# renaudbedard/raytracing-in-one-weekend

Measured on AMD Instinct MI355X. Metric: Msamples/s, 486-sphere cover scene 1920x1080 8-bounce, higher is better.
Workload: dtype f32

## Files before the change

__graft_entry__.py:

```python
import importlib
import os
import subprocess
import sys

ROOT = os.path.dirname(os.path.abspath(__file__))
if ROOT not in sys.path:
    sys.path.insert(0, ROOT)


def build():
    csrc = os.path.join(ROOT, "raytracing-in-one-weekend_amd", "csrc")
    subprocess.run(["make", "-C", csrc], check=True)
    subprocess.run(["make", "-C", os.path.join(ROOT, "oracle")], check=True)
    out_dir = os.path.join(ROOT, "tests", "build")
    os.makedirs(out_dir, exist_ok=True)
    flags = ["-std=c++17", "-O3", "--offload-arch=gfx950", "-ffp-contract=off", "-fno-fast-math", "-Wno-unused-value", "-x", "hip"]
    for name in ("detmath_parity", "exactmath_parity", "exactdiv_parity", "finalize_parity"):
        src, exe = os.path.join(ROOT, "tests", "native", name + ".hip"), os.path.join(out_dir, name)
        deps = [src] + [os.path.join(csrc, h) for h in ("rtow_finalize.hip.h", "rtow_detmath.hip.h", "rtow_exactmath.hip.h")]
        if not os.path.exists(exe) or os.path.getmtime(exe) < max(os.path.getmtime(d) for d in deps):
            subprocess.run(["/opt/rocm/bin/hipcc"] + (flags if name != "detmath_parity" else ["-std=c++17", "-O2", "--offload-arch=gfx950", "-ffp-contract=off", "-fno-fast-math", "-x", "hip"]) + [src, "-o", exe], check=True)
    src, so = os.path.join(ROOT, "tests", "native", "hitsort_parity.hip"), os.path.join(out_dir, "libhitsort_parity.so")
    hdr = os.path.join(ROOT, "raytracing-in-one-weekend_amd", "csrc", "rtow_sample_kernel.hip.h")
    if not os.path.exists(so) or os.path.getmtime(so) < max(os.path.getmtime(src), os.path.getmtime(hdr)):
        subprocess.run(["/opt/rocm/bin/hipcc"] + flags[:-2] + ["-Wno-unused-function", "-fPIC", "-shared", "-x", "hip", src, "-o", so], check=True)
    src, so = os.path.join(ROOT, "tests", "native", "fake_rccl.cpp"), os.path.join(out_dir, "libfake_rccl.so")
    if not os.path.exists(so) or os.path.getmtime(so) < os.path.getmtime(src):
        subprocess.run(["/opt/rocm/bin/hipcc", "-std=c++17", "-O2", "-fPIC", "-shared", "-x", "c++", "-D__HIP_PLATFORM_AMD__", "-I/opt/rocm/include", src, "-o", so,
                        "-L/opt/rocm/lib", "-lamdhip64", "-pthread"], check=True)
    for name in ("valu_calib", "coherence_probe", "sqrt_variants", "xcd_affinity_probe"):
        src, exe = os.path.join(ROOT, "profiles", "calib", name + ".hip"), os.path.join(ROOT, "profiles", "calib", name)
        if not os.path.exists(exe) or os.path.getmtime(exe) < os.path.getmtime(src):
            subprocess.run(["/opt/rocm/bin/hipcc", "-O2"] + flags[2:] + [src, "-o", exe], check=True)
    rt = importlib.import_module("raytracing-in-one-weekend_amd")
    lib = rt.lib.load()
    assert lib.rtowGetApiVersion() == rt.abi.RTOW_API_VERSION
    for name in rt.abi.EXPORTED_SYMBOLS:
        getattr(lib, name)


def smoke():
    import numpy as np

    rt = importlib.import_module("raytracing-in-one-weekend_amd")
    from oracle import binding as ob

    scene = rt.scenes.cover_scene()
    desc = scene.desc()
    params = rt.scenes.make_params(scene, 96, 54, spp=4, trace_depth=8)
    with rt.Context(0) as ctx:
        ctx.upload_scene(desc)
        gpu = rt.sample_batch_host(ctx, params)
        ms = ctx.last_sample_kernel_ms()
    osc = ob.OracleScene(desc)
    ref = osc.sample_batch(params)
    osc.close()
    for k in ("color", "normal", "albedo", "scw"):
        assert np.array_equal(gpu[k].view(np.uint32), ref[k].view(np.uint32)), "smoke: %s differs from the oracle" % k
    assert np.array_equal(gpu["diag"][:, 0], ref["diag"][:, 0]), "smoke: RayCount differs"
    mean = gpu["color"][:, :3] / np.maximum(gpu["color"][:, 3:4], 1)
    mref = ref["color"][:, :3] / np.maximum(ref["color"][:, 3:4], 1)
    assert np.abs(mean - mref).max() <= 1e-4
    plist = [rt.scenes.make_params(scene, 96, 54, spp=4, trace_depth=8, seed=s) for s in (1, 2)]
    n = 96 * 54
    with rt.Context(0) as ctx:
        ctx.upload_scene(desc)
        bufs = [rt.DeviceBuffer(ctx, n * c * 4).zero() for c in (4, 3, 3, 1)]
        rt.lib.check(rt.sample_batch_chain_device(ctx, plist, bufs, bufs), "rtowSampleBatchChainDevice")
        ctx.synchronize()
        chained = {k: b.download(np.float32, (n, c)) for k, b, c in zip(("color", "normal", "albedo", "scw"), bufs, (4, 3, 3, 1))}
    osc = ob.OracleScene(desc)
    ref2 = osc.sample_batch(plist[1], {k: ref[k] for k in ("color", "normal", "albedo", "scw")})
    osc.close()
    for k in ("color", "normal", "albedo", "scw"):
        assert np.array_equal(chained[k].reshape(-1).view(np.uint32), ref2[k].reshape(-1).view(np.uint32)), "smoke: chained %s differs from the oracle" % k
    print("smoke ok: 96x54x4spp cover scene bit-exact vs oracle (single batch and a chain of two), kernel %.3f ms" % ms)


if __name__ == "__main__":
    build()
    if len(sys.argv) > 1 and sys.argv[1] == "smoke":
        smoke()
```

raytracing-in-one-weekend_amd/csrc/rtow_exactmath.hip.h:

```cpp
#pragma once
#include <hip/hip_runtime.h>

namespace rtow {

__device__ __forceinline__ float exact_rcp(float x)
{
    if (__builtin_expect(((__float_as_uint(x) & 0x7f800000u) - 0x01000000u) <= 0x7d000000u, 1)) {
        const float y = __builtin_amdgcn_rcpf(x);
        const float e = __builtin_fmaf(-x, y, 1.0f);
        return __builtin_fmaf(e, y, y);
    }
    return 1.0f / x;
}

__device__ __forceinline__ float exact_rcp_nan_to_inf(float x)
{
    if (__builtin_expect(((__float_as_uint(x) & 0x7f800000u) - 0x01000000u) <= 0x7d000000u, 1)) {
        const float y = __builtin_amdgcn_rcpf(x);
        const float e = __builtin_fmaf(-x, y, 1.0f);
        return __builtin_fmaf(e, y, y);
    }
    const float r = 1.0f / x;
    return r != r ? __builtin_inff() : r;
}

__device__ __forceinline__ float exact_sqrt(float x)
{
    if (__builtin_expect((__float_as_uint(x) - 0x10000000u) < 0x6f000000u, 1)) {
        const float y = __builtin_amdgcn_rsqf(x);
        const float s = x * y;
        const float h = 0.5f * y;
        const float r = __builtin_fmaf(-s, s, x);
        return __builtin_fmaf(r, h, s);
    }
    return __builtin_sqrtf(x);
}

__device__ __forceinline__ float exact_div_step(float a, float b, float y)
{
    const float q = a * y;
    const float r = __builtin_fmaf(-b, q, a);
    return __builtin_fmaf(r, y, q);
}

__device__ __forceinline__ void exact_div3(float ax, float ay, float az, float b, float& qx, float& qy, float& qz)
{
    const unsigned g = ((__float_as_uint(ax) << 1) + 0x40000000u) & ((__float_as_uint(ay) << 1) + 0x40000000u) & ((__float_as_uint(az) << 1) + 0x40000000u);
    const bool bOk = ((__float_as_uint(b) & 0x7f800000u) - 0x30000000u) < 0x20000000u;
    if (__builtin_expect((int)g < 0 && bOk, 1)) {
        const float y0 = __builtin_amdgcn_rcpf(b);
        const float e = __builtin_fmaf(-b, y0, 1.0f);
        const float y = __builtin_fmaf(e, y0, y0);
        qx = exact_div_step(ax, b, y);
        qy = exact_div_step(ay, b, y);
        qz = exact_div_step(az, b, y);
    } else {
        qx = ax / b; qy = ay / b; qz = az / b;
    }
}

__host__ inline float exact_rcp(float x) { return 1.0f / x; }
__host__ inline float exact_rcp_nan_to_inf(float x) { const float r = 1.0f / x; return r != r ? __builtin_inff() : r; }
__host__ inline float exact_sqrt(float x) { return __builtin_sqrtf(x); }
__host__ inline void exact_div3(float ax, float ay, float az, float b, float& qx, float& qy, float& qz) { qx = ax / b; qy = ay / b; qz = az / b; }

}
```

raytracing-in-one-weekend_amd/csrc/rtow_sample_kernel.hip.h:

```cpp
#pragma once
#include "rtow_kernels.h"

#include <type_traits>

#include "rtow_detmath.hip.h"
#include "rtow_hit_tests.hip.h"
#include "rtow_surface.hip.h"
#include "rtow_vecmath.hip.h"

#ifndef RTOW_WHOLE_MATERIAL
#define RTOW_WHOLE_MATERIAL 1
#endif
#ifndef RTOW_LDS_VIEW
#define RTOW_LDS_VIEW 2
#endif
#ifndef RTOW_COLD_VIEW
#define RTOW_COLD_VIEW 1
#endif
#ifndef RTOW_TRI_HOT
#define RTOW_TRI_HOT 1
#endif
#ifndef RTOW_PREFETCH
#define RTOW_PREFETCH 0
#endif
#ifndef RTOW_PINHOLE
#define RTOW_PINHOLE 1
#endif
#ifndef RTOW_TIE_WATCH
#define RTOW_TIE_WATCH 1
#endif

namespace rtow {

namespace {

__device__ __forceinline__ float inv_pow2(int depth)
{
    if (depth <= 126) return __uint_as_float((unsigned)(127 - depth) << 23);
    if (depth == 127) return __uint_as_float(0x00400000u);
    return 0.0f;
}

__device__ __forceinline__ float rng_next(unsigned& state)
{
    const unsigned t = state;
    unsigned s = t;
    s ^= s << 13;
    s ^= s >> 17;
    s ^= s << 5;
    state = s;
    return __uint_as_float(0x3f800000u | (t >> 9)) - 1.0f;
}

__device__ __forceinline__ V3 tangent_to_world(float tx, float ty, float tz, V3 n)
{
    const float s = n.z >= 0 ? 1.0f : -1.0f;
    const float a = -RTOW_RCP(s + n.z);
    const float b = n.x * n.y * a;
    const V3 tangent = v3(1 + s * n.x * n.x * a, s * b, -s * n.x);
    const V3 bitangent = v3(b, s + n.y * n.y * a, -n.y);
    const V3 r = v3(tangent.x * tx + n.x * ty + bitangent.x * tz,
                    tangent.y * tx + n.y * ty + bitangent.y * tz,
                    tangent.z * tx + n.z * ty + bitangent.z * tz);
    return normalize(r);
}
__device__ __forceinline__ V3 cosine_hemisphere_uv(float u, float v, V3 n)
{
    const float radius = RTOW_SQRT(u);
    const float theta = v * 2 * kPi;
    float sinT, cosT;
    det_sincos(theta, sinT, cosT);
    const float tx = radius * cosT, tz = radius * sinT;
    const float ty = RTOW_SQRT(1 - u);
    return tangent_to_world(tx, ty, tz, n);
}
__device__ __forceinline__ V3 direction_uv(float r0, float r1)
{
    const float z = r0 * 2.0f - 1.0f;
    const float rr = RTOW_SQRT(um_max(1.0f - z * z, 0.0f));
    const float angle = r1 * kPi * 2.0f;
    float sn, cs;
    det_sincos(angle, sn, cs);
    return v3(cs * rr, sn * rr, z);
}

struct NoiseSite { const SampleKernelArgs* A; unsigned cx, cy; };

__device__ __forceinline__ unsigned noise_texel(unsigned n, unsigned rowStride, unsigned cx, unsigned cy)
{
    constexpr float g = 1.32471795724474602596f;
    constexpr float a1 = 1.0f / g;
    constexpr float a2 = 1.0f / (g * g);
    const float fn = (float)(n - 1u);
    const float x = 0.5f + a1 * fn, y = 0.5f + a2 * fn;
    const float rx = x - __builtin_floorf(x), ry = y - __builtin_floorf(y);
    const unsigned ox = (unsigned)__builtin_floorf(rx * (float)rowStride), oy = (unsigned)__builtin_floorf(ry * (float)rowStride);
    return ((cy + oy) % rowStride) * rowStride + ((cx + ox) % rowStride);
}

template <int NOISE>
struct Rng;

template <>
struct Rng<RTOW_NOISE_WHITE> {
    unsigned s;
    __device__ __forceinline__ void begin_pixel(const NoiseSite&, unsigned pix, unsigned seed)
    {
        s = (seed * 0x8C4CA03Fu) ^ (pix * 0x7383ED49u);
        (void)rng_next(s);
    }
    __device__ __forceinline__ void begin_sample(const NoiseSite& at, unsigned pix, unsigned smp)
    {
        s = ((at.A->seed * 0x8C4CA03Fu) ^ (pix * 0x7383ED49u)) ^ ((smp + 1u) * 0x9E3779B9u);
        if (s == 0u) s = 0x9E3779B9u;
        (void)rng_next(s);
    }
    __device__ __forceinline__ float next(const NoiseSite&) { return rng_next(s); }
    __device__ __forceinline__ void next2(const NoiseSite&, float& a, float& b) { a = rng_next(s); b = rng_next(s); }
    __device__ __forceinline__ void in_unit_disk(const NoiseSite&, float& x, float& y)
    {
        const float theta = rng_next(s) * (2.0f * kPi - 0.0f) + 0.0f;
        const float radius = RTOW_SQRT(rng_next(s));
        float sinT, cosT;
        det_sincos(theta, sinT, cosT);
        x = radius * cosT; y = radius * sinT;
    }
    __device__ __forceinline__ V3 cosine_hemisphere(const NoiseSite&, V3 n) { const float u = rng_next(s), v = rng_next(s); return cosine_hemisphere_uv(u, v, n); }
    __device__ __forceinline__ void skip_cosine_hemisphere(const NoiseSite&) { (void)rng_next(s); (void)rng_next(s); }
    __device__ __forceinline__ V3 direction(const NoiseSite&) { const float r0 = rng_next(s), r1 = rng_next(s); return direction_uv(r0, r1); }
    __device__ __forceinline__ unsigned trace_value() const { return s; }
};

struct RngPerSample {
    unsigned s, s1;
    __device__ __forceinline__ static unsigned rotl(unsigned x, unsigned k) { return __builtin_amdgcn_alignbit(x, x, 32u - k); }
    __device__ __forceinline__ float draw(const NoiseSite& at)
    {
        if (at.A->xoroshiro) {
            const unsigned s0 = s;
            unsigned t1 = s1;
            const unsigned result = rotl(s0 * 0x9E3779BBu, 5u) * 5u;
            t1 ^= s0;
            s = rotl(s0, 26u) ^ t1 ^ (t1 << 9);
            s1 = rotl(t1, 13u);
            return __uint_as_float(0x3f800000u | (result >> 9)) - 1.0f;
        }
        return rng_next(s);
    }
    __device__ __forceinline__ void begin_pixel(const NoiseSite&, unsigned, unsigned) { s = 1u; s1 = 0u; }
    __device__ __forceinline__ void begin_sample(const NoiseSite& at, unsigned pix, unsigned smp)
    {
        s = ((at.A->seed * 0x8C4CA03Fu) ^ (pix * 0x7383ED49u)) ^ ((smp + 1u) * 0x9E3779B9u);
        if (at.A->xoroshiro) {
            s1 = (s * 0x85EBCA6Bu) ^ 0xC2B2AE35u;
            if ((s | s1) == 0u) s1 = 0x9E3779B9u;
        } else if (s == 0u) {
// ... 540 lines not shown
    int st = ST_REGEN;
    int pix = -1;
    unsigned tick = 0;
    typename std::conditional<PER_SAMPLE && NOISE == RTOW_NOISE_WHITE, RngPerSample, Rng<NOISE>>::type rng{};
    V3 fbNormal = v3(0, 0, 0), fbAlbedo = v3(0, 0, 0);
    unsigned unitGroup = 0;
    unsigned smp = 0, nsamp = 0;
    int cx = 0, cy = 0;
    V3 colorAcc = v3(0, 0, 0), normalAcc = v3(0, 0, 0), albedoAcc = v3(0, 0, 0);
    float scwAcc = 0, scw0 = 0;
    int sampleCount = 0;
    float rayCount = 0, boundsHits = 0, candidates = 0;

    V3 ro = v3(0, 0, 0), rd = v3(0, 0, 1);
    float rtime = 0;
    int depth = 0;
    Hist<HW> hist;
    hist.clear();
    V3 sampleNormal = v3(0, 0, 0);
    int firstNs = -1;
    float randomEventsLocal = 0;

    float texHist[TEXTURED ? HW * 2 * 6 : 1];
    constexpr int kMaxHits = VOLUMES ? kLocalHits : 1;
    float hitT[kMaxHits], hitTmin0[kMaxHits];
    unsigned hitCode[kMaxHits];
    bool tieAtBest = false;
    bool hitOverflow = false;
    int nHits = 0;
    int curVol = -1;
    float pendRE = 0;
    bool insideHit = false;
    float hitTmin = 0;
    constexpr bool TRIANGLES_ONLY = BASE == SCENE_KIND_TRIANGLES || BASE == SCENE_KIND_TRIANGLES_TEXTURED;
    constexpr bool TRI_HOT = TRIANGLES_ONLY && RTOW_TRI_HOT;
    constexpr bool PREFETCH_FAR = WIDE && !ALL_LDS && (RTOW_PREFETCH & 1) != 0;
    constexpr bool PREFETCH_TRI = WIDE && !ALL_LDS && TRI_HOT && (RTOW_PREFETCH & 2) != 0;
    const uint32_t ldsDump __attribute__((unused)) = (uint32_t)(uintptr_t)(__attribute__((address_space(3))) uint8_t*)(smem + ((uint32_t)kCandCapacity + A.ldsStackRows) * (uint32_t)BT * 4u);
    constexpr bool KEEP_NORMAL = BASE == SCENE_KIND_GENERAL || BASE == SCENE_KIND_TRIANGLES;
    V3 keptNormal = v3(0, 0, 0);

    V3 inv = v3(0, 0, 0);
    int cur = 0, sp = 0, nc = 0, prim = -1;
    float best = 0;

    auto endSample = [&](bool ok, V3 sampleColor, V3 skyColor) {
        V3 sampleAlbedo = ok ? skyColor : v3(0, 0, 0);
        if (firstNs >= 0) {
            const unsigned code = hist.get(firstNs, histRows);
            const bool white = (code & 0x8000u) != 0;
            if (TEXTURED) {
                const V3 refl = white ? v3(1, 1, 1) : v3(texHist[firstNs * 6 + 0], texHist[firstNs * 6 + 1], texHist[firstNs * 6 + 2]);
                sampleAlbedo = add(v3(texHist[firstNs * 6 + 3], texHist[firstNs * 6 + 4], texHist[firstNs * 6 + 5]), refl);
            } else {
                const uint8_t* mp = section<ALL_LDS>(sc, L.materialOffset) + (code & 0x7fffu) * 64u;
                const float4 m0 = *reinterpret_cast<const float4*>(mp);
                const float2 m1 = *reinterpret_cast<const float2*>(mp + 16);
                const V3 refl = white ? v3(1, 1, 1) : v3(m0.x, m0.y, m0.z);
                sampleAlbedo = add(v3(m0.w, m1.x, m1.y), refl);
            }
        }
        if (ok) {
            scwAcc += randomEventsLocal;
            colorAcc = add(colorAcc, sampleColor);
            normalAcc = add(normalAcc, sampleNormal);
            albedoAcc = add(albedoAcc, sampleAlbedo);
            sampleCount++;
        } else if (PER_SAMPLE) {
            if (smp == 0) { fbNormal = sampleNormal; fbAlbedo = sampleAlbedo; }
        } else if (smp == 0 && sampleCount == 0 && !A.probeOnly) {
            const SampleKernelArgs& R = A;
            float* fbN = R.outNormal;
            float* fbA = R.outAlbedo;
            if (chained && R.chainIndependent) { fbN = R.chainBatches[tick >> kChainShift].outNormal; fbA = R.chainBatches[tick >> kChainShift].outAlbedo; }
            fbN += 3 * (size_t)pix;
            fbA += 3 * (size_t)pix;
            fbN[0] = sampleNormal.x; fbN[1] = sampleNormal.y; fbN[2] = sampleNormal.z;
            fbA[0] = sampleAlbedo.x; fbA[1] = sampleAlbedo.y; fbA[2] = sampleAlbedo.z;
        }
        smp++;
        st = ST_REGEN;
    };
    auto startRay = [&]() {
        inv = v3(RTOW_RCP_NAN_TO_INF(rd.x), RTOW_RCP_NAN_TO_INF(rd.y), RTOW_RCP_NAN_TO_INF(rd.z));
        cur = 0; sp = 0; nc = 0; prim = -1;
        best = __builtin_inff();
        tieAtBest = false;
        nHits = 0;
        st = ST_TRAV;
        if (DIAG == 2) { if (refDiag) { const float2 rc = reference_counts(A.refTree, ro, rd); boundsHits += rc.x; candidates += rc.y; } }
    };
    auto classify = [&]() {
        rayCount += 1.0f;
        if (VOLUMES) { st = ST_VOL; return; }
        st = prim < 0 ? ST_SKY : ST_HIT;
    };

    uint4 pcand = make_uint4(WIDE ? 0xffffffffu : kNoPrimaryList, 0u, 0u, 0u);
    int force = -1;
    constexpr bool HURRY = RTOW_URGENT_LANES && (GEO & kGeoHurry) != 0;
    unsigned trip = 0;
    STAT_DECL;
    STAGE_DECL;
    for (;;) {
        STAT_ADD(0, 1);
        STAGE_MARK_TOP(7);
        if (chained) { trip++; if ((trip & 7u) == 0u && st == ST_IDLE) st = ST_REGEN; }
        const unsigned long long liveMask = __ballot(st != ST_DEAD && st != ST_IDLE);
        const int live = (int)__popcll(liveMask);
        auto need = [&](int sixtyFourths) { const int t = (live * sixtyFourths + 63) >> 6; return t < 1 ? 1 : t; };
        constexpr unsigned kHurryGrace = 2u;
        unsigned long long hurry = 0ull;
        if (HURRY) hurry = liveMask & __ballot(rayCount > __int_as_float(A.tune[7] & ~255) * (float)(smp + kHurryGrace));
        auto due = [&](bool waiting, int stage, int sixtyFourths) {
            const unsigned long long m = __ballot(waiting);
            return (int)__popcll(m) >= (force == stage ? 1 : need(sixtyFourths)) || (HURRY && (m & hurry) != 0ull);
        };
        bool ran = false;
        constexpr bool PIXEL_COMPANY = HW == 32 || PER_SAMPLE;
        bool regenReady = st == ST_REGEN;
        const int pixelGate = HURRY ? A.tune[7] & 255 : A.tune[7];
        if (PIXEL_COMPANY && pixelGate > 1) {
            const int wantPixel = (int)__popcll(__ballot(st == ST_REGEN && smp >= nsamp));
            const int company = live < pixelGate ? live : pixelGate;
            if (wantPixel < company && force != ST_REGEN) regenReady = st == ST_REGEN && (smp < nsamp || (HURRY && ((hurry >> (tid & 63)) & 1ull) != 0ull));
        }
        if (due(regenReady, ST_REGEN, A.tune[0])) {
            ran = true;
            STAGE_MARK(0);
            STAT_ADD(1, 1);
            if (regenReady) {
                STAT_LANES(2);
                while (smp >= nsamp) {
#if defined(__HIP_DEVICE_COMPILE__)
                    const SampleKernelArgs* coldArgs = (const SampleKernelArgs*)__builtin_amdgcn_kernarg_segment_ptr();
                    asm volatile("" : "+s"(coldArgs));
#else
                    const SampleKernelArgs* coldArgs = &A;
#endif
                    const SampleKernelArgs& C = *coldArgs;
                    const bool grouped = chained && C.chainIndependent != 0;
                    const bool redo = REDO_CAPABLE && C.redoMode != 0;
                    const unsigned tk = chained ? (tick & kChainTicketMask) : tick;
                    const unsigned batch = chained ? (tick >> kChainShift) : 0u;
                    if (pix >= 0 && C.pixelCost) {
                        const unsigned rc = (unsigned)rayCount;
                        C.pixelCost[tk] = (unsigned short)(rc < 65535u ? rc : 65535u);
                    }
                    if (VOLUMES && hitOverflow) { *C.overflowFlag = 1u; hitOverflow = false; }
                    if (pix >= 0 && C.probeOnly) pix = -1;
                    bool redoContinue = false;
                    if (PER_SAMPLE && pix >= 0) {
                        const bool fallback = unitGroup == 0 && sampleCount == 0;
                        float4* rec = reinterpret_cast<float4*>(C.unitRecords) + (size_t)tick * 4u;
                        rec[0] = make_float4(colorAcc.x, colorAcc.y, colorAcc.z, (float)sampleCount);
                        rec[1] = fallback ? make_float4(fbNormal.x, fbNormal.y, fbNormal.z, rayCount) : make_float4(normalAcc.x, normalAcc.y, normalAcc.z, rayCount);
                        rec[2] = fallback ? make_float4(fbAlbedo.x, fbAlbedo.y, fbAlbedo.z, scwAcc) : make_float4(albedoAcc.x, albedoAcc.y, albedoAcc.z, scwAcc);
                        rec[3] = make_float4(boundsHits, candidates, 0, 0);
                        pix = -1;
                    }
                    if (pix >= 0 && chained) {
                        float *oc = C.outColor, *on = C.outNormal, *oa = C.outAlbedo, *os = C.outScw;
                        if (grouped) { const ChainBatch cb = C.chainBatches[batch]; oc = cb.outColor; on = cb.outNormal; oa = cb.outAlbedo; os = cb.outScw; }
                        reinterpret_cast<float4*>(oc)[pix] = make_float4(colorAcc.x, colorAcc.y, colorAcc.z, (float)sampleCount);
                        if (sampleCount != 0 || nsamp == 0) {
                            const V3 nrm = sampleCount != 0 ? normalAcc : v3(0, 0, 0), alb = sampleCount != 0 ? albedoAcc : v3(0, 0, 0);
                            on[3 * (size_t)pix + 0] = nrm.x; on[3 * (size_t)pix + 1] = nrm.y; on[3 * (size_t)pix + 2] = nrm.z;
// ... 137 lines not shown
                                if (waveQueue[2] != 0u) { parked = true; break; }
                                __builtin_amdgcn_fence(__ATOMIC_ACQUIRE, "workgroup");
                            }
                        }
                        const unsigned take = (unsigned)__popcll(need) < end - next ? (unsigned)__popcll(need) : end - next;
                        if ((unsigned)rank < take) { ticket = next + (unsigned)rank; got = true; }
                        if (lane == leader) waveQueue[0] = next + take;
                    }
                    if (ticket == 0xffffffffu) { st = parked ? ST_IDLE : ST_DEAD; break; }
                    if (REDO_CAPABLE) { if (redo) ticket = C.tieRedo[4u + ticket]; }
                    if (grouped && !redo) {
                        const unsigned slot = ticket >> 6;
                        const unsigned place = __umulhi(slot, C.groupRecip);
                        const unsigned chunk = C.chunkOrder ? C.chunkOrder[place] : place;
                        ticket = (chunk << 6) | (ticket & 63u);
                        if (ticket >= C.totalWork) { pix = -1; nsamp = 0; smp = 0; continue; }
                        ticket |= (slot - place * C.chainCount) << kChainShift;
                    }
                    tick = ticket;
                    newBatch = chained ? (ticket >> kChainShift) : 0u;
                    if (chained) ticket &= kChainTicketMask;
                    if (PER_SAMPLE) { unitGroup = ticket % C.groupsPerPixel; ticket = ticket / C.groupsPerPixel; }
                    else if (!(REDO_CAPABLE && redo)) { const unsigned* const map = C.ticketMap; if (map && ticket < C.tiledPixels) ticket = map[ticket]; }
                    int ownedRow;
                    owned_pixel_xy(ticket, (unsigned)C.width, C.tilesPerRow, C.tiledPixels, cx, ownedRow);
                    cy = C.sliceOffset + ownedRow * C.sliceDivider;
                    if (REDO_CAPABLE) { if (redo) { cy = (int)(ticket / (unsigned)C.width); cx = (int)(ticket - (unsigned)cy * (unsigned)C.width); } }
                    pix = cy * C.width + cx;

                    float4 last = make_float4(0, 0, 0, 0);
                    if (PER_SAMPLE) {
                        last.w = C.inColor[4 * (size_t)pix + 3];
                        scwAcc = C.inScw[pix];
                    } else if (chained && !grouped && !redo) {
                        const float* ic = (newBatch == 0u ? C.inColor : C.outColor) + 4 * (size_t)pix;
                        const float* in_ = (newBatch == 0u ? C.inNormal : C.outNormal) + 3 * (size_t)pix;
                        const float* ia = (newBatch == 0u ? C.inAlbedo : C.outAlbedo) + 3 * (size_t)pix;
                        last = coherent_load4(ic);
                        normalAcc = coherent_load3(in_);
                        albedoAcc = coherent_load3(ia);
                        scwAcc = coherent_load((newBatch == 0u ? C.inScw : C.outScw) + pix);
                    } else if (!C.probeOnly) {
                        last = reinterpret_cast<const float4*>(C.inColor)[pix];
                        normalAcc = v3(C.inNormal[3 * (size_t)pix], C.inNormal[3 * (size_t)pix + 1], C.inNormal[3 * (size_t)pix + 2]);
                        albedoAcc = v3(C.inAlbedo[3 * (size_t)pix], C.inAlbedo[3 * (size_t)pix + 1], C.inAlbedo[3 * (size_t)pix + 2]);
                        scwAcc = C.inScw[pix];
                    }
                    colorAcc = v3(last.x, last.y, last.z);
                    sampleCount = (int)last.w;
                    }
                    const float scwIn = scwAcc;
                    const int countIn = sampleCount;

                    rng.begin_pixel(NoiseSite{&A, (unsigned)cx, (unsigned)cy}, (unsigned)pix, chained ? C.chainBatches[newBatch].seed : C.seed);

                    const float w = scwIn / (float)countIn;
                    if (w == 0) {
                        nsamp = C.sampleCountMin;
                    } else {
                        const RtowFloat2* const fed = chained ? C.chainBatches[newBatch].extrema : C.extremaIn;
                        const float ex = fed ? fed->x : C.extremaX, ey = fed ? fed->y : C.extremaY;
                        const float nw = um_saturate((w - ex) / (ey - ex));
                        const float lo = (float)C.sampleCountMin, hi = (float)C.sampleCountMax;
                        nsamp = (unsigned)__builtin_rintf(lo + nw * (hi - lo));
                    }
                    if (C.probeOnly) nsamp = (unsigned)C.probeOnly;
                    scw0 = w;
                    smp = 0;
                    if (PER_SAMPLE) {
                        smp = unitGroup * kSampleGroup;
                        nsamp = nsamp < smp + kSampleGroup ? nsamp : smp + kSampleGroup;
                        if (nsamp < smp) nsamp = smp;
                        colorAcc = v3(0, 0, 0); normalAcc = v3(0, 0, 0); albedoAcc = v3(0, 0, 0);
                        sampleCount = 0;
                        scwAcc = 0;
                    }
                    rayCount = 0; boundsHits = 0; candidates = 0;
                    if (WIDE || LONG_LISTS) pcand = C.pixelCandidates ? reinterpret_cast<const uint4*>(C.pixelCandidates)[pix] : make_uint4(WIDE ? 0xffffffffu : kNoPrimaryList, 0u, 0u, 0u);
                    else { const uint2 pc = C.pixelCandidates ? C.pixelCandidates[2 * (size_t)pix] : make_uint2(kNoPrimaryList, 0u); pcand = make_uint4(pc.x, pc.y, 0u, 0u); }
                }
                if (st == ST_REGEN) {
                    const SampleKernelArgs& VA = COLD_VIEW ? cold_args(A) : A;
                    const RtowView& VW = LDS_VIEW ? *reinterpret_cast<const RtowView*>(ldsConst) : VA.view;
                    const float frameX = LDS_VIEW ? ldsConst[29] : VA.sizeX, frameY = LDS_VIEW ? ldsConst[30] : VA.sizeY;
                    const V3 viewRight = PINHOLE ? v3(0, 0, 0) : v3(VW.right), viewUp = PINHOLE ? v3(0, 0, 0) : v3(VW.up);
                    const V3 viewLLC = v3(VW.lowerLeftCorner), viewH = v3(VW.horizontal), viewV = v3(VW.vertical);
                    const float lensRadius = PINHOLE ? 0.0f : VW.lensRadius;
                    float jx = 0.5f, jy = 0.5f;
                    const NoiseSite at{&A, (unsigned)cx, (unsigned)cy};
                    if (PER_SAMPLE) rng.begin_sample(at, (unsigned)pix, smp);
                    if (A.subPixelJitter) rng.next2(at, jx, jy);
                    const float u = ((float)cx + jx) / frameX;
                    const float v = ((float)cy + jy) / frameY;
                    float rdx = 0, rdy = 0;
                    if (lensRadius != 0) {
                        float dx, dy;
                        rng.in_unit_disk(at, dx, dy);
                        rdx = lensRadius * dx;
                        rdy = lensRadius * dy;
                    }
                    const V3 offset = v3(viewRight.x * rdx + viewUp.x * rdy, viewRight.y * rdx + viewUp.y * rdy, viewRight.z * rdx + viewUp.z * rdy);
                    ro = add(v3(VW.origin), offset);
                    rd = normalize(v3(viewLLC.x - offset.x + u * viewH.x + v * viewV.x,
                                      viewLLC.y - offset.y + u * viewH.y + v * viewV.y,
                                      viewLLC.z - offset.z + u * viewH.z + v * viewV.z));
                    rtime = rng.next(at);
                    if (HAS_MOTION) { if (L.commonTimeRange) rtime = um_max(0.0f, um_min(1.0f, (rtime - L.commonT0) / (L.commonT1 - L.commonT0))); }

                    depth = 0;
                    hist.clear();
                    sampleNormal = v3(0, 0, 0);
                    firstNs = -1;
                    randomEventsLocal = 0;
                    curVol = -1;
                    pendRE = 0;
                    startRay();
                    if (WIDE ? !(pcand.x == 0xffffffffu && pcand.y != 0xffffffffu) : pcand.x != kNoPrimaryList) {
                        const f2 invx = {inv.x, inv.x}, invy = {inv.y, inv.y}, invz = {inv.z, inv.z};
                        const f2 ox = {ro.x, ro.x}, oy = {ro.y, ro.y}, oz = {ro.z, ro.z};
                        cur = -1;
                        for (int k = 0; k < 4; k++) {
                            const unsigned node = WIDE ? (k == 0 ? pcand.x : k == 1 ? pcand.y : k == 2 ? pcand.z : pcand.w)
                                                       : ((k < 2 ? pcand.x >> (16 * k) : pcand.y >> (16 * (k - 2))) & 0xffffu);
                            if (node == (WIDE ? 0xffffffffu : 0xffffu)) break;
                            float4 q0, q1, q2;
                            int c0, c1;
                            load_node<ALL_LDS, SPLIT_NODES>(sc, L, (int)node, q0, q1, q2, c0, c1);
                            const f2 tlx = (f2{q0.x, q0.y} - ox) * invx, thx = (f2{q1.z, q1.w} - ox) * invx;
                            const f2 tly = (f2{q0.z, q0.w} - oy) * invy, thy = (f2{q2.x, q2.y} - oy) * invy;
                            const f2 tlz = (f2{q1.x, q1.y} - oz) * invz, thz = (f2{q2.z, q2.w} - oz) * invz;
                            const float tmin0 = vmax3(vmin(tlx.x, thx.x), vmin(tly.x, thy.x), vmax(vmin(tlz.x, thz.x), 0.0f));
                            const float tfar0 = vmin3(vmax(tlx.x, thx.x), vmax(tly.x, thy.x), vmax(tlz.x, thz.x));
                            const float tmin1 = vmax3(vmin(tlx.y, thx.y), vmin(tly.y, thy.y), vmax(vmin(tlz.y, thz.y), 0.0f));
                            const float tfar1 = vmin3(vmax(tlx.y, thx.y), vmax(tly.y, thy.y), vmax(tlz.y, thz.y));
                            const bool leaf0 = c0 < 0 && tmin0 < tfar0;
                            const bool leaf1 = c1 < 0 && tmin1 < tfar1 && twoChildren;
                            if (FULL_DIAG && !refDiag) boundsHits += (leaf0 ? 1.0f : 0.0f) + (leaf1 ? 1.0f : 0.0f);
                            cand[nc * BT] = (Code)~c0;
                            nc += leaf0 ? 1 : 0;
                            cand[nc * BT] = (Code)~c1;
                            nc += leaf1 ? 1 : 0;
                        }
                        if (LONG_LISTS) { if ((pcand.z & 0xffffu) != 0xffffu) cur = -6; }
                        if (nc == 0 && cur == -1) classify(); else st = ST_TEST;
                    }
                }
            }
        }
        if (due(st == ST_TRAV, ST_TRAV, A.tune[1])) {
            ran = true;
            STAGE_MARK(1);
            if (st == ST_TRAV) {
                const f2 invx = {inv.x, inv.x}, invy = {inv.y, inv.y}, invz = {inv.z, inv.z};
                const f2 ox = {ro.x, ro.x}, oy = {ro.y, ro.y}, oz = {ro.z, ro.z};
                int budget = A.travSlice;
                const float bestPrune = best * 1.000244140625f;
                const int candExit = VOLUMES ? kCandCapacity - 2 : (A.tune[6] < kCandCapacity - 1 ? A.tune[6] : kCandCapacity - 1) - 1;
                while (budget > 0 && cur >= 0 && nc <= candExit) {
                    budget--;
                    STAT_ADD(3, (threadIdx.x & 63) == __builtin_ctzll(__ballot(1)) ? 1 : 0);
                    STAT_LANES(4);
                    float4 q0, q1, q2;
                    int c0, c1;
                    load_node<ALL_LDS, SPLIT_NODES>(sc, L, cur, q0, q1, q2, c0, c1);
                    const int spm1 = sp > 0 ? sp - 1 : 0;
                    const int popped = (int)stack[spm1 * BT];
                    const f2 tlx = (f2{q0.x, q0.y} - ox) * invx, thx = (f2{q1.z, q1.w} - ox) * invx;
                    const f2 tly = (f2{q0.z, q0.w} - oy) * invy, thy = (f2{q2.x, q2.y} - oy) * invy;
                    const f2 tlz = (f2{q1.x, q1.y} - oz) * invz, thz = (f2{q2.z, q2.w} - oz) * invz;
                    const float tmin0 = vmax3(vmin(tlx.x, thx.x), vmin(tly.x, thy.x), vmax(vmin(tlz.x, thz.x), 0.0f));
                    const float tfar0 = vmin3(vmax(tlx.x, thx.x), vmax(tly.x, thy.x), vmax(tlz.x, thz.x));
                    const float tmin1 = vmax3(vmin(tlx.y, thx.y), vmin(tly.y, thy.y), vmax(vmin(tlz.y, thz.y), 0.0f));
                    const float tfar1 = vmin3(vmax(tlx.y, thx.y), vmax(tly.y, thy.y), vmax(tlz.y, thz.y));
                    const bool hit0 = tmin0 <= vmin(tfar0, bestPrune);
                    const bool hit1 = tmin1 <= vmin(tfar1, bestPrune) && twoChildren;
                    const bool leaf0 = c0 < 0 && hit0 && tmin0 < tfar0, leaf1 = c1 < 0 && hit1 && tmin1 < tfar1;
                    if (FULL_DIAG && !refDiag) boundsHits += ((c0 < 0 ? leaf0 : hit0) ? 1.0f : 0.0f) + ((c1 < 0 ? leaf1 : hit1) ? 1.0f : 0.0f);
                    cand[nc * BT] = (Code)~c0;
                    nc += leaf0 ? 1 : 0;
                    cand[nc * BT] = (Code)~c1;
                    nc += leaf1 ? 1 : 0;
                    if (PREFETCH_TRI) {
                        if (leaf0) prefetch_sector(sc.glob, L.triHotOffset + (uint32_t)~c0 * (uint32_t)sizeof(GpuTriHot), ldsDump);
                        if (leaf1) prefetch_sector(sc.glob, L.triHotOffset + (uint32_t)~c1 * (uint32_t)sizeof(GpuTriHot), ldsDump);
                    }
// ... 383 lines not shown
                                        if (!(tn < tf)) continue;
                                    }
                                    float t; V3 nl; float4 rq;
                                    if (general_hit<ALL_LDS>(sc, L, ~cc, mw >> kPrimTypeShift, ro, bd, rtime, 0.0f, t, nl, rq) && dot(normalize(rotate(rq, nl)), bd) > 0) insideVolume = true;
                                }
                                const bool in0 = h0 && c0 >= 0, in1 = h1 && c1 >= 0;
                                if (in0 && in1) { stack[bsp * BT] = (Code)c1; bsp++; bcur = c0; }
                                else if (in0 || in1) bcur = in0 ? c0 : c1;
                                else if (bsp > 0) { bsp--; bcur = (int)stack[bsp * BT]; }
                                else bcur = -1;
                            }
                            if (insideVolume) { curVol = (int)(matOf(c) & 0xffffu); break; }
                        }
                    }
                    for (int i = 0; i < nHits; i++) DBG_TRACE(10 + i, codeAt(i), distAt(i));
                    DBG_TRACE(9, 0, 0.0f);
                    int hitIndex = 0;
                    int chosen = -1;
                    insideHit = false;
                    while (hitIndex < nHits) {
                        const unsigned c = codeAt(hitIndex);
                        const unsigned mw = matOf(c);
                        if (curVol >= 0 || ((mw >> 16) & 3u) == MAT_CLASS_VOLUME) {
                            const bool isEntryHit = curVol < 0;
                            if (curVol < 0) curVol = (int)(mw & 0xffffu);
                            int exitHitIndex = hitIndex, lastExitIndex = -1, sameMaterialEntries = 0;
                            while (exitHitIndex < nHits) {
                                const unsigned ec = codeAt(exitHitIndex);
                                if ((int)(matOf(ec) & 0xffffu) == curVol) {
                                    if (ec & 0x40000000u) sameMaterialEntries++;
                                    else { sameMaterialEntries--; lastExitIndex = exitHitIndex; }
                                    if (sameMaterialEntries <= 0) break;
                                } else
                                    break;
                                exitHitIndex++;
                            }
                            if (sameMaterialEntries > 0 && lastExitIndex != -1) exitHitIndex = lastExitIndex;
                            if (exitHitIndex < nHits) {
                                float distanceInVolume = distAt(exitHitIndex);
                                float entryDistance = 0;
                                if (isEntryHit) { entryDistance = distAt(hitIndex); distanceInVolume -= distAt(hitIndex); }
                                const float density = *reinterpret_cast<const float*>(section<ALL_LDS>(sc, L.materialOffset) + (unsigned)curVol * 64u + 36u);
                                pendRE++;
                                const float volumeHitDistance = -(RTOW_RCP(um_max(density, 1.1920928955078125e-7f))) * det_log(rng.next(NoiseSite{&A, (unsigned)cx, (unsigned)cy}));
                                if (volumeHitDistance < distanceInVolume) {
                                    best = entryDistance + volumeHitDistance;
                                    insideHit = true;
                                    break;
                                }
                                curVol = -1;
                                const unsigned xc = codeAt(exitHitIndex);
                                if (isVolume(xc) && (xc & 0x80000000u)) { hitIndex = exitHitIndex + 1; continue; }
                                chosen = exitHitIndex;
                                break;
                            }
                            nHits = 0;
                            break;
                        }
                        chosen = hitIndex;
                        break;
                    }
                    if (insideHit) { prim = -1; st = ST_HIT; }
                    else if (chosen >= 0 && chosen < nHits) { best = distAt(chosen); hitTmin = tminAt(chosen); prim = (int)(codeAt(chosen) & kHitPrimMask); st = ST_HIT; }
                    else st = ST_SKY;
                };
                const HitSpill spill = hit_spill_of(A);
                if (nHits > kMaxHits) sort_hit_list_spilled(hitT, hitTmin0, hitCode, spill, nHits, reinterpret_cast<const unsigned*>(section<ALL_LDS>(sc, L.rankOffset)));
                else if (nHits > 1) sort_hit_list(hitT, hitTmin0, hitCode, nHits, reinterpret_cast<const unsigned*>(section<ALL_LDS>(sc, L.rankOffset)));
                volumeLogic([&](int i) { return hit_get(hitT, hitTmin0, hitCode, spill, i).t; }, [&](int i) { return hit_get(hitT, hitTmin0, hitCode, spill, i).code; },
                            [&](int i) { return hit_get(hitT, hitTmin0, hitCode, spill, i).tmin0; });
            }
        }
        if (due(st == ST_SKY, ST_SKY, A.tune[4])) {
            ran = true;
            STAGE_MARK(4);
            STAT_ADD(15, 1);
            if (st == ST_SKY) {
                DBG_TRACE(2, 0xffff, 0.0f);
                V3 sky = v3(0, 0, 0);
                const SampleKernelArgs& EA = COLD_VIEW ? cold_args(A) : A;
                const RtowEnvironment& ENV = LDS_VIEW ? *reinterpret_cast<const RtowEnvironment*>(ldsConst + 22) : EA.environment;
                if (ENV.skyType == RTOW_SKY_GRADIENT) {
                    const float s = 0.5f * (rd.y + 1);
                    const V3 b = v3(ENV.skyBottomColor), tp = v3(ENV.skyTopColor);
                    sky = v3(b.x + s * (tp.x - b.x), b.y + s * (tp.y - b.y), b.z + s * (tp.z - b.z));
                } else if (ENV.skyType == RTOW_SKY_CUBEMAP) {
                    sky = cubemap_sample(cold_args(A).cubemap, rd);
                }
                if (VOLUMES) { randomEventsLocal += pendRE * inv_pow2(depth); pendRE = 0; }
                if (firstNs < 0) sampleNormal = neg(rd);

                V3 col = sky;
                for (int i = depth - 1; i >= 0; i--) {
                    const unsigned code = hist.get(i, histRows);
                    const uint8_t* mp = section<ALL_LDS>(sc, L.materialOffset) + (code & 0x7fffu) * 64u;
                    const float4 m0 = *reinterpret_cast<const float4*>(mp);
                    const float2 m1 = *reinterpret_cast<const float2*>(mp + 16);
                    const bool white = (code & 0x8000u) != 0;
                    if (TEXTURED) {
                        const V3 att = white ? v3(1, 1, 1) : v3(texHist[i * 6 + 0], texHist[i * 6 + 1], texHist[i * 6 + 2]);
                        col = v3(col.x * att.x + texHist[i * 6 + 3], col.y * att.y + texHist[i * 6 + 4], col.z * att.z + texHist[i * 6 + 5]);
                        continue;
                    }
                    const unsigned wmask = (unsigned)((int)(code << 16) >> 31);
                    auto pick = [&](float albedo) { return __uint_as_float((__float_as_uint(albedo) & ~wmask) | (0x3f800000u & wmask)); };
                    const V3 att = v3(pick(m0.x), pick(m0.y), pick(m0.z));
                    col = v3(col.x * att.x + m0.w, col.y * att.y + m1.x, col.z * att.z + m1.y);
                }
                endSample(true, col, sky);
            }
        }
        STAGE_MARK(7);
        if (ran) {
            force = -1;
        } else {
            int top = 0;
            force = -1;
            for (int k = ST_REGEN; k < ST_COUNT; k++) {
                const int n = (int)__popcll(__ballot(st == k));
                if (n > top) { top = n; force = k; }
            }
            if (top == 0) {
                if (!chained || __ballot(st == ST_IDLE) == 0ull) break;
                __builtin_amdgcn_s_sleep(64);
                if (st == ST_IDLE) st = ST_REGEN;
                force = ST_REGEN;
            }
        }
    }
}

template <bool ALL_LDS, int KIND, int HW, int DIAG, int NOISE, bool PER_SAMPLE, int GEO = 0>
hipError_t launchVariant(const SampleKernelArgs& args, int numBlocks, hipStream_t stream)
{
    auto k = sample_batch_kernel<ALL_LDS, KIND, HW, DIAG, NOISE, PER_SAMPLE, GEO>;
    const size_t ldsBytes = (size_t)args.ldsFrontBytes + (size_t)kQueueBytes + args.ldsSceneBytes;
    if (args.ldsStackRows < 1u || ldsBytes > (size_t)kLdsBytesMax) return hipErrorInvalidValue;
    if (HW == 32 && args.traceDepth > kHistoryInRegisters) {
        const uint32_t rows = (uint32_t)(args.traceDepth - kHistoryInRegisters);
        if ((args.ldsHistRows > 0u && args.ldsHistOffset == 0u) || (args.ldsHistRows < rows && (ALL_LDS || !args.histSpill || args.histSpillRows < rows - args.ldsHistRows))) return hipErrorInvalidValue;
    }
    hipError_t e = hipFuncSetAttribute(reinterpret_cast<const void*>(k), hipFuncAttributeMaxDynamicSharedMemorySize, (int)ldsBytes);
    if (e != hipSuccess) return e;
    hipLaunchKernelGGL(k, dim3(numBlocks), dim3(geo_block_threads(GEO)), ldsBytes, stream, args);
    return hipGetLastError();
}

template <int KIND>
constexpr bool kTiesWithShortHistory = true;

template <bool ALL_LDS, int KIND, int GEO>
hipError_t launchByDiagGeo(const SampleKernelArgs& args, int numBlocks, hipStream_t stream)
{
    constexpr bool TIES = (KIND & kExactTiesBit) != 0;
    constexpr bool WIDE = (GEO & kGeoWide) != 0;
    const bool fullDiag = args.diagnostics && args.diagnosticsStride >= 16;
    const int hw = historyWords(args.noiseColor, args.unitRecords != nullptr, WIDE, TIES, fullDiag, args.traceDepth);
    constexpr bool HAS_HURRY_TWIN = RTOW_URGENT_LANES && !WIDE && !TIES && (KIND & 7) == SCENE_KIND_SPHERES;
    const bool hurry = ((uint32_t)args.tune[7] >> 8) != 0u;
    if (hurry && !hurryTwin(KIND & 7, TIES, WIDE, args.noiseColor, args.unitRecords != nullptr, fullDiag, args.refTree != nullptr, args.traceDepth)) return hipErrorInvalidValue;
    if (args.noiseColor == RTOW_NOISE_BLUE) return launchVariant<ALL_LDS, KIND, 32, 2, RTOW_NOISE_BLUE, false, GEO>(args, numBlocks, stream);
    if (args.noiseColor == RTOW_NOISE_SPATIOTEMPORAL_BLUE) return launchVariant<ALL_LDS, KIND, 32, 2, RTOW_NOISE_SPATIOTEMPORAL_BLUE, false, GEO>(args, numBlocks, stream);
    if (args.unitRecords) {
        if constexpr (!TIES && !WIDE) if (hw == 4) return launchVariant<ALL_LDS, KIND, 4, 0, RTOW_NOISE_WHITE, true, GEO>(args, numBlocks, stream);
        return launchVariant<ALL_LDS, KIND, 32, 2, RTOW_NOISE_WHITE, true, GEO>(args, numBlocks, stream);
    }
    constexpr bool HAS_PINHOLE_TWIN = RTOW_PINHOLE && !ALL_LDS && !WIDE && (KIND & 7) == SCENE_KIND_SPHERES;
// ... 44 lines not shown
```

raytracing-in-one-weekend_amd/csrc/rtow_vecmath.hip.h:

```cpp
#pragma once
#include <hip/hip_runtime.h>

#include "../../include/rtow.h"
#include "rtow_exactmath.hip.h"

#ifndef RTOW_EXACT_MATH
#define RTOW_EXACT_MATH 1
#endif
#if RTOW_EXACT_MATH
#define RTOW_RCP(x) rtow::exact_rcp(x)
#define RTOW_RCP_NAN_TO_INF(x) rtow::exact_rcp_nan_to_inf(x)
#define RTOW_SQRT(x) rtow::exact_sqrt(x)
#ifndef RTOW_EXACT_DIV3
#define RTOW_EXACT_DIV3 1
#endif
#else
#define RTOW_RCP(x) (1.0f / (x))
#define RTOW_RCP_NAN_TO_INF(x) ([](float r_) { return r_ != r_ ? __builtin_inff() : r_; }(1.0f / (x)))
#define RTOW_SQRT(x) __builtin_sqrtf(x)
#define RTOW_EXACT_DIV3 0
#endif

namespace rtow {

namespace {

struct V3 { float x, y, z; };

__host__ __device__ __forceinline__ V3 v3(float x, float y, float z) { V3 r; r.x = x; r.y = y; r.z = z; return r; }
__host__ __device__ __forceinline__ V3 v3(const RtowFloat3& a) { return v3(a.x, a.y, a.z); }
__host__ __device__ __forceinline__ V3 add(V3 a, V3 b) { return v3(a.x + b.x, a.y + b.y, a.z + b.z); }
__host__ __device__ __forceinline__ V3 sub(V3 a, V3 b) { return v3(a.x - b.x, a.y - b.y, a.z - b.z); }
__host__ __device__ __forceinline__ V3 neg(V3 a) { return v3(-a.x, -a.y, -a.z); }
__host__ __device__ __forceinline__ V3 scale(float s, V3 a) { return v3(s * a.x, s * a.y, s * a.z); }
__host__ __device__ __forceinline__ float dot(V3 a, V3 b) { return a.x * b.x + a.y * b.y + a.z * b.z; }
__device__ __forceinline__ V3 normalize(V3 v) { const float r = RTOW_RCP(RTOW_SQRT(dot(v, v))); return scale(r, v); }
__device__ __forceinline__ V3 reflect(V3 i, V3 n)
{
    const float d = dot(i, n);
    return v3(i.x - (2.0f * n.x) * d, i.y - (2.0f * n.y) * d, i.z - (2.0f * n.z) * d);
}
__host__ __device__ __forceinline__ float um_min(float x, float y) { return (y != y || x < y) ? x : y; }
__host__ __device__ __forceinline__ float um_max(float x, float y) { return (y != y || x > y) ? x : y; }
__device__ __forceinline__ float um_saturate(float x) { return um_max(0.0f, um_min(1.0f, x)); }

constexpr float kPi = 3.14159265f;

__device__ __forceinline__ float half_bits_to_float(unsigned h)
{
    const unsigned sign = (h & 0x8000u) << 16;
    const unsigned exp = (h >> 10) & 0x1fu, man = h & 0x3ffu;
    if (exp == 0) return __uint_as_float(__float_as_uint((float)man * 5.9604644775390625e-8f) | sign);
    if (exp == 31) return __uint_as_float(sign | 0x7f800000u | (man << 13));
    return __uint_as_float(sign | ((exp + 112u) << 23) | (man << 13));
}

__host__ __device__ __forceinline__ V3 div3(V3 p, float d)
{
#if RTOW_EXACT_DIV3
    V3 q;
    rtow::exact_div3(p.x, p.y, p.z, d, q.x, q.y, q.z);
    return q;
#else
    return v3(p.x / d, p.y / d, p.z / d);
#endif
}

__host__ __device__ __forceinline__ V3 cross(V3 a, V3 b) { return v3(a.y * b.z - a.z * b.y, a.z * b.x - a.x * b.z, a.x * b.y - a.y * b.x); }
__host__ __device__ __forceinline__ V3 rotate(float4 q, V3 v)
{
    const V3 qv = v3(q.x, q.y, q.z);
    const V3 t = scale(2.0f, cross(qv, v));
    const V3 c = cross(qv, t);
    return v3(v.x + q.w * t.x + c.x, v.y + q.w * t.y + c.y, v.z + q.w * t.z + c.z);
}
__host__ __device__ __forceinline__ float um_sign(float x) { return (x > 0.0f ? 1.0f : 0.0f) - (x < 0.0f ? 1.0f : 0.0f); }

}

}
```

Before: 9564.

## Fuse exact-math range checks and pin view constants in scalar registers

Adds fused exact-math helpers (rcp3, sqrt2, div2, rcp_sqrt) that share a single range-check branch across multiple lanes of math instead of branching per scalar op. These are used in normalize, ray start, cosine hemisphere sampling and camera ray generation. Camera and sky constants are also packed into vector types and pinned into SGPRs with empty asm constraints, so they are not reloaded or moved to VGPRs. This is meant to reduce branch and VALU overhead while keeping bit-exact results, at the cost of added register pressure and asm hints that could constrain the compiler.

Result: faster. 9662 (median of 6 runs) (+1.0%).

```diff
diff --git a/__graft_entry__.py b/__graft_entry__.py
--- a/__graft_entry__.py
+++ b/__graft_entry__.py
@@ -15,7 +15,7 @@
     out_dir = os.path.join(ROOT, "tests", "build")
     os.makedirs(out_dir, exist_ok=True)
     flags = ["-std=c++17", "-O3", "--offload-arch=gfx950", "-ffp-contract=off", "-fno-fast-math", "-Wno-unused-value", "-x", "hip"]
-    for name in ("detmath_parity", "exactmath_parity", "exactdiv_parity", "finalize_parity"):
+    for name in ("detmath_parity", "exactmath_parity", "exactdiv_parity", "exactmath_fused_parity", "finalize_parity"):
         src, exe = os.path.join(ROOT, "tests", "native", name + ".hip"), os.path.join(out_dir, name)
         deps = [src] + [os.path.join(csrc, h) for h in ("rtow_finalize.hip.h", "rtow_detmath.hip.h", "rtow_exactmath.hip.h")]
         if not os.path.exists(exe) or os.path.getmtime(exe) < max(os.path.getmtime(d) for d in deps):
diff --git a/raytracing-in-one-weekend_amd/csrc/rtow_exactmath.hip.h b/raytracing-in-one-weekend_amd/csrc/rtow_exactmath.hip.h
--- a/raytracing-in-one-weekend_amd/csrc/rtow_exactmath.hip.h
+++ b/raytracing-in-one-weekend_amd/csrc/rtow_exactmath.hip.h
@@ -59,6 +59,65 @@
     }
 }
 
+
+__device__ __forceinline__ void exact_rcp3_nan_to_inf(float x, float y, float z, float& rx, float& ry, float& rz)
+{
+    const unsigned g = ((__float_as_uint(x) << 1) + 0x40000000u) & ((__float_as_uint(y) << 1) + 0x40000000u) & ((__float_as_uint(z) << 1) + 0x40000000u);
+    if (__builtin_expect((int)g < 0, 1)) {
+        const float x0 = __builtin_amdgcn_rcpf(x), y0 = __builtin_amdgcn_rcpf(y), z0 = __builtin_amdgcn_rcpf(z);
+        const float ex = __builtin_fmaf(-x, x0, 1.0f), ey = __builtin_fmaf(-y, y0, 1.0f), ez = __builtin_fmaf(-z, z0, 1.0f);
+        rx = __builtin_fmaf(ex, x0, x0);
+        ry = __builtin_fmaf(ey, y0, y0);
+        rz = __builtin_fmaf(ez, z0, z0);
+    } else {
+        rx = exact_rcp_nan_to_inf(x); ry = exact_rcp_nan_to_inf(y); rz = exact_rcp_nan_to_inf(z);
+    }
+}
+
+__device__ __forceinline__ float exact_rcp_sqrt(float d)
+{
+    if (__builtin_expect((__float_as_uint(d) - 0x10000000u) < 0x6f000000u, 1)) {
+        const float y = __builtin_amdgcn_rsqf(d);
+        const float s0 = d * y;
+        const float h = 0.5f * y;
+        const float r = __builtin_fmaf(-s0, s0, d);
+        const float s = __builtin_fmaf(r, h, s0);
+        const float w = __builtin_amdgcn_rcpf(s);
+        const float e = __builtin_fmaf(-s, w, 1.0f);
+        return __builtin_fmaf(e, w, w);
+    }
+    return exact_rcp(__builtin_sqrtf(d));
+}
+
+__device__ __forceinline__ void exact_sqrt2(float a, float b, float& sa, float& sb)
+{
+    const unsigned ka = __float_as_uint(a) - 0x10000000u, kb = __float_as_uint(b) - 0x10000000u;
+    if (__builtin_expect((ka > kb ? ka : kb) < 0x6f000000u, 1)) {
+        const float ya = __builtin_amdgcn_rsqf(a), yb = __builtin_amdgcn_rsqf(b);
+        const float s0 = a * ya, s1 = b * yb;
+        const float ha = 0.5f * ya, hb = 0.5f * yb;
+        const float ra = __builtin_fmaf(-s0, s0, a), rb = __builtin_fmaf(-s1, s1, b);
+        sa = __builtin_fmaf(ra, ha, s0);
+        sb = __builtin_fmaf(rb, hb, s1);
+    } else {
+        sa = exact_sqrt(a); sb = exact_sqrt(b);
+    }
+}
+
+__device__ __forceinline__ void exact_div2(float ax, float bx, float ay, float by, float& qx, float& qy)
+{
+    const unsigned g = ((__float_as_uint(ax) << 1) + 0x40000000u) & ((__float_as_uint(ay) << 1) + 0x40000000u);
+    const bool bOk = ((__float_as_uint(bx) & 0x7f800000u) - 0x30000000u) < 0x20000000u && ((__float_as_uint(by) & 0x7f800000u) - 0x30000000u) < 0x20000000u;
+    if (__builtin_expect((int)g < 0 && bOk, 1)) {
+        const float x0 = __builtin_amdgcn_rcpf(bx), y0 = __builtin_amdgcn_rcpf(by);
+        const float ex = __builtin_fmaf(-bx, x0, 1.0f), ey = __builtin_fmaf(-by, y0, 1.0f);
+        qx = exact_div_step(ax, bx, __builtin_fmaf(ex, x0, x0));
+        qy = exact_div_step(ay, by, __builtin_fmaf(ey, y0, y0));
+    } else {
+        qx = ax / bx; qy = ay / by;
+    }
+}
+
 __host__ inline float exact_rcp(float x) { return 1.0f / x; }
 __host__ inline float exact_rcp_nan_to_inf(float x) { const float r = 1.0f / x; return r != r ? __builtin_inff() : r; }
 __host__ inline float exact_sqrt(float x) { return __builtin_sqrtf(x); }
diff --git a/raytracing-in-one-weekend_amd/csrc/rtow_sample_kernel.hip.h b/raytracing-in-one-weekend_amd/csrc/rtow_sample_kernel.hip.h
--- a/raytracing-in-one-weekend_amd/csrc/rtow_sample_kernel.hip.h
+++ b/raytracing-in-one-weekend_amd/csrc/rtow_sample_kernel.hip.h
@@ -66,12 +66,12 @@
 }
 __device__ __forceinline__ V3 cosine_hemisphere_uv(float u, float v, V3 n)
 {
-    const float radius = RTOW_SQRT(u);
+    float radius, ty;
+    RTOW_SQRT2(u, 1 - u, radius, ty);
     const float theta = v * 2 * kPi;
     float sinT, cosT;
     det_sincos(theta, sinT, cosT);
     const float tx = radius * cosT, tz = radius * sinT;
-    const float ty = RTOW_SQRT(1 - u);
     return tangent_to_world(tx, ty, tz, n);
 }
 __device__ __forceinline__ V3 direction_uv(float r0, float r1)
@@ -778,7 +778,7 @@
         st = ST_REGEN;
     };
     auto startRay = [&]() {
-        inv = v3(RTOW_RCP_NAN_TO_INF(rd.x), RTOW_RCP_NAN_TO_INF(rd.y), RTOW_RCP_NAN_TO_INF(rd.z));
+        RTOW_RCP3_NAN_TO_INF(rd.x, rd.y, rd.z, inv.x, inv.y, inv.z);
         cur = 0; sp = 0; nc = 0; prim = -1;
         best = __builtin_inff();
         tieAtBest = false;
@@ -1082,16 +1082,32 @@
                 if (st == ST_REGEN) {
                     const SampleKernelArgs& VA = COLD_VIEW ? cold_args(A) : A;
                     const RtowView& VW = LDS_VIEW ? *reinterpret_cast<const RtowView*>(ldsConst) : VA.view;
-                    const float frameX = LDS_VIEW ? ldsConst[29] : VA.sizeX, frameY = LDS_VIEW ? ldsConst[30] : VA.sizeY;
-                    const V3 viewRight = PINHOLE ? v3(0, 0, 0) : v3(VW.right), viewUp = PINHOLE ? v3(0, 0, 0) : v3(VW.up);
-                    const V3 viewLLC = v3(VW.lowerLeftCorner), viewH = v3(VW.horizontal), viewV = v3(VW.vertical);
-                    const float lensRadius = PINHOLE ? 0.0f : VW.lensRadius;
+                    typedef float sf4 __attribute__((ext_vector_type(4)));
+                    typedef float sf2 __attribute__((ext_vector_type(2)));
+                    sf4 k0 = {VW.origin.x, VW.origin.y, VW.origin.z, VW.lowerLeftCorner.x};
+                    sf4 k1 = {VW.lowerLeftCorner.y, VW.lowerLeftCorner.z, VW.horizontal.x, VW.horizontal.y};
+                    sf4 k2 = {VW.horizontal.z, VW.vertical.x, VW.vertical.y, VW.vertical.z};
+                    sf4 k3 = {0, 0, 0, 0};
+                    sf2 k4 = {0, 0};
+                    float k5 = 0;
+                    sf2 kf = {LDS_VIEW ? ldsConst[29] : VA.sizeX, LDS_VIEW ? ldsConst[30] : VA.sizeY};
+                    if (!PINHOLE) { k3 = sf4{VW.up.x, VW.up.y, VW.up.z, VW.right.x}; k4 = sf2{VW.right.y, VW.right.z}; k5 = VW.lensRadius; }
+                    if (LDS_VIEW) asm volatile("" : "+v"(kf));
+                    if (!LDS_VIEW && !COLD_VIEW) {
+                        if (PINHOLE) asm volatile("" : "+s"(k0), "+s"(k1), "+s"(k2), "+s"(kf));
+                        else asm volatile("" : "+s"(k0), "+s"(k1), "+s"(k2), "+s"(k3), "+s"(k4), "+s"(k5), "+s"(kf));
+                    }
+                    const V3 viewOrigin = v3(k0.x, k0.y, k0.z);
+                    const V3 viewRight = v3(k3.w, k4.x, k4.y), viewUp = v3(k3.x, k3.y, k3.z);
+                    const V3 viewLLC = v3(k0.w, k1.x, k1.y), viewH = v3(k1.z, k1.w, k2.x), viewV = v3(k2.y, k2.z, k2.w);
+                    const float lensRadius = k5;
+                    const float frameX = kf.x, frameY = kf.y;
                     float jx = 0.5f, jy = 0.5f;
                     const NoiseSite at{&A, (unsigned)cx, (unsigned)cy};
                     if (PER_SAMPLE) rng.begin_sample(at, (unsigned)pix, smp);
                     if (A.subPixelJitter) rng.next2(at, jx, jy);
-                    const float u = ((float)cx + jx) / frameX;
-                    const float v = ((float)cy + jy) / frameY;
+                    float u, v;
+                    RTOW_DIV2((float)cx + jx, frameX, (float)cy + jy, frameY, u, v);
                     float rdx = 0, rdy = 0;
                     if (lensRadius != 0) {
                         float dx, dy;
@@ -1100,7 +1116,7 @@
                         rdy = lensRadius * dy;
                     }
                     const V3 offset = v3(viewRight.x * rdx + viewUp.x * rdy, viewRight.y * rdx + viewUp.y * rdy, viewRight.z * rdx + viewUp.z * rdy);
-                    ro = add(v3(VW.origin), offset);
+                    ro = add(viewOrigin, offset);
                     rd = normalize(v3(viewLLC.x - offset.x + u * viewH.x + v * viewV.x,
                                       viewLLC.y - offset.y + u * viewH.y + v * viewV.y,
                                       viewLLC.z - offset.z + u * viewH.z + v * viewV.z));
@@ -1650,7 +1666,12 @@
                 const RtowEnvironment& ENV = LDS_VIEW ? *reinterpret_cast<const RtowEnvironment*>(ldsConst + 22) : EA.environment;
                 if (ENV.skyType == RTOW_SKY_GRADIENT) {
                     const float s = 0.5f * (rd.y + 1);
-                    const V3 b = v3(ENV.skyBottomColor), tp = v3(ENV.skyTopColor);
+                    typedef float sf4 __attribute__((ext_vector_type(4)));
+                    typedef float sf2 __attribute__((ext_vector_type(2)));
+                    sf4 e0 = {ENV.skyBottomColor.x, ENV.skyBottomColor.y, ENV.skyBottomColor.z, ENV.skyTopColor.x};
+                    sf2 e1 = {ENV.skyTopColor.y, ENV.skyTopColor.z};
+                    if (!LDS_VIEW && !COLD_VIEW) asm volatile("" : "+s"(e0), "+s"(e1));
+                    const V3 b = v3(e0.x, e0.y, e0.z), tp = v3(e0.w, e1.x, e1.y);
                     sky = v3(b.x + s * (tp.x - b.x), b.y + s * (tp.y - b.y), b.z + s * (tp.z - b.z));
                 } else if (ENV.skyType == RTOW_SKY_CUBEMAP) {
                     sky = cubemap_sample(cold_args(A).cubemap, rd);
diff --git a/raytracing-in-one-weekend_amd/csrc/rtow_vecmath.hip.h b/raytracing-in-one-weekend_amd/csrc/rtow_vecmath.hip.h
--- a/raytracing-in-one-weekend_amd/csrc/rtow_vecmath.hip.h
+++ b/raytracing-in-one-weekend_amd/csrc/rtow_vecmath.hip.h
@@ -11,6 +11,10 @@
 #define RTOW_RCP(x) rtow::exact_rcp(x)
 #define RTOW_RCP_NAN_TO_INF(x) rtow::exact_rcp_nan_to_inf(x)
 #define RTOW_SQRT(x) rtow::exact_sqrt(x)
+#define RTOW_RCP_SQRT(x) rtow::exact_rcp_sqrt(x)
+#define RTOW_RCP3_NAN_TO_INF(x, y, z, rx, ry, rz) rtow::exact_rcp3_nan_to_inf(x, y, z, rx, ry, rz)
+#define RTOW_SQRT2(a, b, sa, sb) rtow::exact_sqrt2(a, b, sa, sb)
+#define RTOW_DIV2(ax, bx, ay, by, qx, qy) rtow::exact_div2(ax, bx, ay, by, qx, qy)
 #ifndef RTOW_EXACT_DIV3
 #define RTOW_EXACT_DIV3 1
 #endif
@@ -18,6 +22,10 @@
 #define RTOW_RCP(x) (1.0f / (x))
 #define RTOW_RCP_NAN_TO_INF(x) ([](float r_) { return r_ != r_ ? __builtin_inff() : r_; }(1.0f / (x)))
 #define RTOW_SQRT(x) __builtin_sqrtf(x)
+#define RTOW_RCP_SQRT(x) (1.0f / __builtin_sqrtf(x))
+#define RTOW_RCP3_NAN_TO_INF(x, y, z, rx, ry, rz) ((rx) = RTOW_RCP_NAN_TO_INF(x), (ry) = RTOW_RCP_NAN_TO_INF(y), (rz) = RTOW_RCP_NAN_TO_INF(z))
+#define RTOW_SQRT2(a, b, sa, sb) ((sa) = __builtin_sqrtf(a), (sb) = __builtin_sqrtf(b))
+#define RTOW_DIV2(ax, bx, ay, by, qx, qy) ((qx) = (ax) / (bx), (qy) = (ay) / (by))
 #define RTOW_EXACT_DIV3 0
 #endif
 
@@ -34,7 +42,7 @@
 __host__ __device__ __forceinline__ V3 neg(V3 a) { return v3(-a.x, -a.y, -a.z); }
 __host__ __device__ __forceinline__ V3 scale(float s, V3 a) { return v3(s * a.x, s * a.y, s * a.z); }
 __host__ __device__ __forceinline__ float dot(V3 a, V3 b) { return a.x * b.x + a.y * b.y + a.z * b.z; }
-__device__ __forceinline__ V3 normalize(V3 v) { const float r = RTOW_RCP(RTOW_SQRT(dot(v, v))); return scale(r, v); }
+__device__ __forceinline__ V3 normalize(V3 v) { const float r = RTOW_RCP_SQRT(dot(v, v)); return scale(r, v); }
 __device__ __forceinline__ V3 reflect(V3 i, V3 n)
 {
     const float d = dot(i, n);
```
